# mxy-kit/poisson-ellipse-openmp-mpi-cuda-new

Measured on AMD Instinct MI355X. Metric: grid-point updates/sec (MLUPS) + iters-to-tol, 16384^2 grid at 1/2/4/8 MI355X, higher is better.
Workload: dtype fp64; 1 GPU; model=fictitious-domain Poisson ellipse, Jacobi-PCG, 16384x16384, global_batch=1, seq_len=268402689, parallelism=single, split=auto, comm=self, rccl_graph=False, split_sweep=False, kernel=wave, graph_batch=32, overlap=on, exact=False

## Files before the change

### poisson-ellipse-openmp-mpi-cuda-new_amd/csrc/hip/ca_kernels.hip

```cpp
#include <algorithm>
#include <cmath>
#include <type_traits>
#include <utility>
#include <vector>

#include "pcg1_march.hpp"
#include "pcg_device.hpp"
#include "pmx/common.hpp"
#include "pmx/kernels.hpp"
#include "pmx/spec.hpp"

namespace pmx {

using namespace dev;

namespace {

template <int S>
struct CaShape {
  static constexpr int NB = 2 * S + 1;
  static constexpr int NQ = 6 * S;
  static constexpr int NN = S;
  static constexpr int HE = (S + 1) & ~1;
  static constexpr int WO = 128 - 2 * HE;
  static constexpr int AGES = S + 1 > 3 ? S + 1 : 3;
};

template <int S>
__host__ __device__ constexpr int ca_prod_i(int q) {
  if (q <= 2 * S) return q <= S ? q : (q + 1) / 2;
  q -= 2 * S + 1;
  if (q <= 2 * S - 2) return S + 1 + (q <= S - 1 ? q : (q + 1) / 2);
  q -= 2 * S - 1;
  return q <= S ? q : S;
}
template <int S>
__host__ __device__ constexpr int ca_prod_j(int q) {
  if (q <= 2 * S) return q <= S ? 0 : q / 2;
  q -= 2 * S + 1;
  if (q <= 2 * S - 2) return S + 1 + (q <= S - 1 ? 0 : q / 2);
  q -= 2 * S - 1;
  return q <= S ? S + 1 : S + 1 + (q - S);
}

struct CaK {
  double cxh, cyh, d_in, d_out;
};

__device__ __forceinline__ CaK ca_consts(const DevGeom& G) {
  CaK k;
  const double den = 2.0 * (G.cx + G.cy);
  k.cxh = G.cx / den;
  k.cyh = G.cy / den;
  k.d_in = diag<false>(1.0, 1.0, 1.0, 1.0, G);
  k.d_out = diag<false>(G.inv_eps, G.inv_eps, G.inv_eps, G.inv_eps, G);
  return k;
}

template <typename T>
__device__ __forceinline__ const T* ca_col(const T* row, int c) {
  return reinterpret_cast<const T*>(reinterpret_cast<const char*>(row - 8) + unsigned(c + 8) * unsigned(sizeof(T)));
}
template <typename T>
__device__ __forceinline__ T* ca_col(T* row, int c) {
  return reinterpret_cast<T*>(reinterpret_cast<char*>(row - 8) + unsigned(c + 8) * unsigned(sizeof(T)));
}

template <typename T>
__device__ __forceinline__ void ca_load2(const T* row, int c, int cmax, T (&out)[2]) {
  vload_raw<T, 2>(ca_col(row, min(c, cmax)), out);
}

template <typename T>
__device__ __forceinline__ void ca_store2(T* row, int c, const T (&in)[2], bool all, const bool (&own)[2]) {
  typedef T V __attribute__((ext_vector_type(2)));
  if (all) {
    const V v = {in[0], in[1]};
    __builtin_nontemporal_store(v, reinterpret_cast<V*>(ca_col(row, c)));
  } else {
#pragma unroll
    for (int u = 0; u < 2; ++u)
      if (own[u]) __builtin_nontemporal_store(in[u], ca_col(row, c + u));
  }
}

constexpr int kCaRowOff = 8;

__device__ __forceinline__ int ca_row_cls(const unsigned* tbl, int m) {
  const int r = m + kCaRowOff;
  const unsigned wd = ld_uniform(tbl, r >> 4);
  return int((wd >> (2 * (r & 15))) & 3u);
}

struct CaFaces {
  const double* a;
  const double* b;
  int gh;
};

__device__ __forceinline__ int ca_cmax(const DevGeom& G, const CaFaces& F) {
  return (G.nb & kNbYhi) ? ((G.ny + F.gh - 1) | 1) : G.ny + 1 + (G.ny & 1);
}

__device__ __forceinline__ void ca_faces(const CaFaces& F, const DevGeom& G, int r, int c0, int cmax,
                                         double (&a0)[2], double (&a1)[2], double (&b0)[2], double (&b1)[2]) {
  const int rc = min(max(r, 1 - F.gh), G.nx + F.gh - 1);
  const double* ra = F.a + int64_t(rc) * G.pitch;
  const double* rb = F.b + int64_t(rc) * G.pitch;
  vload<double, 2>(ca_col(ra, min(c0, cmax)), a0);
  vload<double, 2>(ca_col(ra + G.pitch, min(c0, cmax)), a1);
  vload<double, 2>(ca_col(rb, min(c0, cmax)), b0);
  b1[0] = b0[1];
  b1[1] = *ca_col(rb, min(c0 + 2, cmax + 1));
}

__device__ __forceinline__ void ca_lt(int ucls, int r, const double (&c)[2], const double (&im)[2],
                                      const double (&ip)[2], double left, double right, const CaK& K,
                                      const DevGeom& G, const CaFaces& F, int c0, int cmax, double (&out)[2]) {
  const double jm[2] = {left, c[0]}, jp[2] = {c[1], right};
  if (ucls != 0) {
#pragma unroll
    for (int u = 0; u < 2; ++u) out[u] = -__builtin_fma(K.cyh, jm[u] + jp[u], K.cxh * (im[u] + ip[u]));
    return;
  }
  double a0[2], a1[2], b0[2], b1[2];
  ca_faces(F, G, r, c0, cmax, a0, a1, b0, b1);
#pragma unroll
  for (int u = 0; u < 2; ++u) {
    if (a0[u] == a1[u] && a0[u] == b0[u] && a0[u] == b1[u]) {
      out[u] = -__builtin_fma(K.cyh, jm[u] + jp[u], K.cxh * (im[u] + ip[u]));
    } else {
      const double av = apply_a<false>(c[u], im[u], ip[u], jm[u], jp[u], a0[u], a1[u], b0[u], b1[u], G);
      out[u] = av / diag<false>(a0[u], a1[u], b0[u], b1[u], G) - c[u];
    }
  }
}

__device__ __forceinline__ void ca_diag(int ucls, int r, const CaK& K, const DevGeom& G, const CaFaces& F, int c0,
                                        int cmax, double (&d)[2]) {
  if (ucls != 0) {
    d[0] = d[1] = ucls == 1 ? K.d_in : K.d_out;
    return;
  }
  double a0[2], a1[2], b0[2], b1[2];
  ca_faces(F, G, r, c0, cmax, a0, a1, b0, b1);
#pragma unroll
  for (int u = 0; u < 2; ++u) d[u] = diag<false>(a0[u], a1[u], b0[u], b1[u], G);
}

template <int CTRL>
__device__ __forceinline__ double dpp_shift0(double v) {
  const long long b = __double_as_longlong(v);
  const int lo = __builtin_amdgcn_mov_dpp(int(b), CTRL, 0xf, 0xf, true);
  const int hi = __builtin_amdgcn_mov_dpp(int(b >> 32), CTRL, 0xf, 0xf, true);
  return __longlong_as_double((long long)(unsigned)lo | ((long long)hi << 32));
}


__host__ __device__ inline bool ca_tile_fast(const DevGeom& G, int i0, int i1, int j0, int j1, int r, int he, int wo) {
  return j1 == j0 + wo - 1 && G.gi0 + i0 - r >= 1 && G.gi0 + i1 + r <= G.M - 1 && G.gj0 + j0 - he >= 1 &&
         G.gj0 + j0 - he + 127 <= G.N - 1;
}

template <int S, int sl>
__device__ __forceinline__ void ca_gather(const double (&XP)[S + 1][4][2], const double (&XZ)[S][4][2],
                                          double (&Y)[CaShape<S>::NB][2]) {
#pragma unroll
  for (int l = 0; l <= S; ++l) {
    Y[l][0] = XP[l][sl][0];
    Y[l][1] = XP[l][sl][1];
  }
#pragma unroll
  for (int l = 0; l < S; ++l) {
    Y[S + 1 + l][0] = XZ[l][sl][0];
    Y[S + 1 + l][1] = XZ[l][sl][1];
  }
}

template <int NB>
__device__ __forceinline__ double ca_dot(const double (&c)[NB], const double (&Y)[NB][2], int u, double v0) {
#pragma unroll
  for (int i = 0; i < NB; ++i) v0 = __builtin_fma(c[i], Y[i][u], v0);
  return v0;
}

template <int S, int N>
__device__ __forceinline__ void ca_norms(const double (&pa)[S][CaShape<S>::NB], const double (&Y)[CaShape<S>::NB][2],
                                         int u, double (&acc)[N]) {
  acc[0] = __builtin_fma(Y[0][u], Y[0][u], acc[0]);
#pragma unroll
  for (int j = 1; j < S; ++j) {
    double v = 0.0;
#pragma unroll
    for (int i = 0; i <= j; ++i) v = __builtin_fma(pa[j][i], Y[i][u], v);
#pragma unroll
    for (int i = 0; i < j; ++i) v = __builtin_fma(pa[j][S + 1 + i], Y[S + 1 + i][u], v);
    acc[j] = __builtin_fma(v, v, acc[j]);
  }
}

template <typename T, int S, bool UPD>
struct CaRow {
  T p[2], z[2], w[2];
};

template <typename T, int S, bool UPD, bool FAST, int PF, bool REW, int DPF = 0, int HE = CaShape<S>::HE>
__device__ __forceinline__ void ca_march(const DevGeom& G, const DevTables& Tb, const CaK& K,
                                         const T* __restrict__ pin, const T* __restrict__ zin, T* __restrict__ pout,
                                         T* __restrict__ zout, T* __restrict__ w, int i0, int i1, int j0, int j1,
                                         const unsigned* __restrict__ ctbl, const CaFaces& F,
                                         double (&acc)[CaShape<S>::NQ], const double (&ca)[CaShape<S>::NB],
                                         const double (&cb)[CaShape<S>::NB], const double (&cc)[CaShape<S>::NB],
                                         const double (&pa)[S][CaShape<S>::NB], double* dring = nullptr) {
  using Sh = CaShape<S>;
  constexpr int NB = Sh::NB;
  const int64_t P = G.pitch;
  const int lane = threadIdx.x & 63;
  const int c0 = j0 - HE + 2 * lane;
  const int cmax = ca_cmax(G, F);
  bool colin[2], own[2];
#pragma unroll
  for (int u = 0; u < 2; ++u) {
    const int c = c0 + u, g = G.gj0 + c;
    colin[u] = g >= 1 && g <= G.N - 1;
    own[u] = c >= j0 && c <= j1;
  }
  const bool own_all = own[0] && own[1];
  const bool own_any = own[0] || own[1];
  auto interior_row = [&](int m) { return G.gi0 + m >= 1 && G.gi0 + m <= G.M - 1; };

  auto fetch = [&](int m, CaRow<T, S, UPD>& b) {
    const int mc = min(max(m, 1 - F.gh), G.nx + F.gh);
    ca_load2<T>(pin + int64_t(mc) * P, c0, cmax, b.p);
    ca_load2<T>(zin + int64_t(mc) * P, c0, cmax, b.z);
    if constexpr (UPD) {
      const int wc = min(max(m - S, 1 - F.gh), G.nx + F.gh);
      ca_load2<T>(w + int64_t(wc) * P, c0, cmax, b.w);
    }
  };

  static_assert(Sh::AGES <= 4, "ca_march: window deeper than 4 rows");
  double XP[S + 1][4][2], XZ[S][4][2];
#pragma unroll
  for (int l = 0; l <= S; ++l)
#pragma unroll
    for (int a = 0; a < 4; ++a) XP[l][a][0] = XP[l][a][1] = 0.0;
#pragma unroll
  for (int l = 0; l < S; ++l)
#pragma unroll
    for (int a = 0; a < 4; ++a) XZ[l][a][0] = XZ[l][a][1] = 0.0;
  int ch[4] = {0, 0, 0, 0};

  const int mfirst = i0 - S, mlast = i1 + S;
  auto level = [&](auto& X, auto lc, auto qc, int m) {
    constexpr int l = decltype(lc)::value, q = decltype(qc)::value;
    constexpr int sc = (q - l) & 3, sm = (q - l - 1) & 3, sp = (q - l + 1) & 3;
    const int r = m - l;
    const double(&ctr)[2] = X[l - 1][sc];
    const double left = dpp_shift0<kWaveShr1>(ctr[1]);
    const double right = dpp_shift0<kWaveShl1>(ctr[0]);
    double lt[2];
    ca_lt(ch[sc], r, ctr, X[l - 1][sm], X[l - 1][sp], left, right, K, G, F, c0, cmax, lt);
    const bool rin = FAST || interior_row(r);
#pragma unroll
    for (int u = 0; u < 2; ++u) {
      double v;
      if constexpr (l == 1) v = lt[u];
      else v = __builtin_fma(2.0, lt[u], -X[l - 2][sc][u]);
      X[l][sc][u] = (FAST || (rin && colin[u])) ? v : 0.0;
    }
  };

  auto core = [&](auto qc, int m, const CaRow<T, S, UPD>& cur) {
    constexpr int q = decltype(qc)::value;
    ch[q] = ca_row_cls(ctbl, m);
    const bool rin = FAST || interior_row(m);
#pragma unroll
    for (int u = 0; u < 2; ++u) {
      const bool in = FAST || (rin && colin[u]);
      XP[0][q][u] = in ? double(cur.p[u]) : 0.0;
      XZ[0][q][u] = in ? double(cur.z[u]) : 0.0;
    }
    static_for_while<S>([&](auto l1) {
      level(XP, std::integral_constant<int, decltype(l1)::value + 1>{}, qc, m);
      return true;
    });
    static_for_while<S - 1>([&](auto l1) {
      level(XZ, std::integral_constant<int, decltype(l1)::value + 1>{}, qc, m);
      return true;
    });
    const int g = m - S;
    if (g < i0 || g > i1) return;
    constexpr int sg = (q - S) & 3;
    double Y[NB][2];
    ca_gather<S, sg>(XP, XZ, Y);
    if constexpr (!UPD) {
      double d[2];
      ca_diag(ch[sg], g, K, G, F, c0, cmax, d);
#pragma unroll
      for (int u = 0; u < 2; ++u) {
        if (!(FAST || own[u])) continue;
#pragma unroll
        for (int q = 0; q < Sh::NQ; ++q)
          acc[q] = __builtin_fma(Y[ca_prod_i<S>(q)][u], d[u] * Y[ca_prod_j<S>(q)][u], acc[q]);
      }
    } else {
      T pn[2], zn[2], wn[2];
#pragma unroll
      for (int u = 0; u < 2; ++u) {
        const double sp = REW ? 0.0 : ca_dot(ca, Y, u, 0.0), sz = REW ? 0.0 : ca_dot(cb, Y, u, 0.0);
        const double sw = ca_dot(cc, Y, u, double(cur.w[u]));
        pn[u] = static_cast<T>(sp);
        zn[u] = static_cast<T>(sz);
        wn[u] = static_cast<T>(sw);
        if constexpr (!REW) {
          if (FAST || own[u]) ca_norms<S>(pa, Y, u, acc);
        }
      }
      if (FAST ? own_all : own_any) {
        const int64_t o = int64_t(g) * P;
        if constexpr (!REW) {
          ca_store2<T>(pout + o, c0, pn, FAST || own_all, own);
          ca_store2<T>(zout + o, c0, zn, FAST || own_all, own);
        }
        ca_store2<T>(w + o, c0, wn, FAST || own_all, own);
      }
    }
  };

  static_assert(PF == 1 || PF == 3, "ca_march: prefetch depth 1 or 3");
  if constexpr (DPF > 0) {
    static_assert(DPF == 4 && !UPD && FAST && sizeof(T) == 8, "ca_march: LDS-DMA for pass 1 FAST tiles, 4 rows");
    const unsigned voff = unsigned(c0 + 4) * 8u;
    const unsigned lds0 = unsigned(reinterpret_cast<uintptr_t>(dring));
    auto dma_row = [&](int m, int slot) {
      const unsigned l = lds0 + unsigned(slot) * 2048u;
      asm volatile("s_waitcnt lgkmcnt(0)" ::: "memory");
      dma16(pin + int64_t(m) * P - 4, voff, l);
      dma16(zin + int64_t(m) * P - 4, voff, l + 1024u);
    };
    typedef double d2 __attribute__((ext_vector_type(2)));
#pragma unroll
    for (int q = 0; q < DPF; ++q) dma_row(min(mfirst + q, mlast), q);
    bool more = true;
    for (int m = mfirst; more && m <= mlast; m += 4) {
      more = static_for_while<4>([&](auto qc) {
        constexpr int q = decltype(qc)::value;
        if (m + q > mlast) return false;
        wait_vmcnt<(DPF - 1) * 2>();
        const double* sl = dring + q * 256;
        CaRow<T, S, UPD> cur;
        const d2 pv = *reinterpret_cast<const d2*>(sl + 2 * lane);
        const d2 zv = *reinterpret_cast<const d2*>(sl + 128 + 2 * lane);
        cur.p[0] = pv.x;
        cur.p[1] = pv.y;
        cur.z[0] = zv.x;
        cur.z[1] = zv.y;
        dma_row(min(m + q + DPF, mlast), q);
        core(qc, m + q, cur);
        return true;
      });
    }
    wait_vmcnt<0>();
    if constexpr (FAST) {
#pragma unroll
      for (int q = 0; q < Sh::NQ; ++q) acc[q] = own_all ? acc[q] : 0.0;
    }
    return;
  }
  constexpr int NBUF = PF + 1;
  CaRow<T, S, UPD> buf[NBUF];
#pragma unroll
  for (int q = 0; q < PF; ++q) fetch(min(mfirst + q, mlast), buf[q]);
  bool more = true;
  for (int m = mfirst; more && m <= mlast; m += 4) {
    more = static_for_while<4>([&](auto qc) {
      constexpr int q = decltype(qc)::value;
      if (m + q > mlast) return false;
      fetch(min(m + q + PF, mlast), buf[(q + PF) % NBUF]);
      core(qc, m + q, buf[q % NBUF]);
      return true;
    });
  }
  if constexpr (FAST) {
#pragma unroll
    for (int q = 0; q < Sh::NQ; ++q) acc[q] = own_all ? acc[q] : 0.0;
  }
}

constexpr int kCaPfGram = 3, kCaPfUpd = 1, kCaPfFuse = 1;

struct CaPart {
  int part;
  int tiles_i, ti_lo, ti_hi, tj_lo, tj_hi;
};

__device__ __forceinline__ void ca_part_tile(int k, const CaPart& P, int tiles_j, int& ti, int& tj) {
  if (P.part == 0) {
    ti = k / tiles_j;
    tj = k - ti * tiles_j;
    return;
  }
  const int h = P.ti_hi - P.ti_lo, wj = P.tj_hi - P.tj_lo;
  if (P.part == 1) {
    ti = P.ti_lo + k / wj;
    tj = P.tj_lo + k % wj;
    return;
  }
  const int ntop = P.ti_lo * tiles_j;
  if (k < ntop) { ti = k / tiles_j; tj = k % tiles_j; return; }
  k -= ntop;
  const int nbot = (P.tiles_i - P.ti_hi) * tiles_j;
  if (k < nbot) { ti = P.ti_hi + k / tiles_j; tj = k % tiles_j; return; }
  k -= nbot;
  if (k < h * P.tj_lo) { ti = P.ti_lo + k / P.tj_lo; tj = k % P.tj_lo; return; }
  k -= h * P.tj_lo;
  const int wr = tiles_j - P.tj_hi;
  ti = P.ti_lo + k / wr;
  tj = P.tj_hi + k % wr;
}

template <typename T, int S, bool UPD, int MW, bool DMA, int PART>
__global__ void __launch_bounds__(64, MW)
k_ca_sweep(DevGeom G, DevTables Tb, T* w, T* z0, T* z1, T* p0, T* p1, double* __restrict__ partials,
           const PcgState* St, const CaState* C, int TI, int tiles_j, const unsigned* __restrict__ ctbl,
           int cwords, int64_t pbase, CaFaces faces, CaPart part, int ntiles) {
  using Sh = CaShape<S>;
  constexpr int NB = Sh::NB;
  typedef const __attribute__((address_space(4))) PcgState CPS;
  typedef const __attribute__((address_space(4))) CaState CCS;
  const int done = ((CPS*)St)->done;
  const long long blk = ((CCS*)C)->blk;
  const int nupd = ((CCS*)C)->nupd;
  double ca[NB], cb[NB], cc[NB], pa[S][NB];
#pragma unroll
  for (int i = 0; i < NB; ++i) {
    ca[i] = UPD ? ((CCS*)C)->coef[0][i] : 0.0;
    cb[i] = UPD ? ((CCS*)C)->coef[1][i] : 0.0;
    cc[i] = UPD ? ((CCS*)C)->coef[2][i] : 0.0;
#pragma unroll
    for (int j = 0; j < S; ++j) pa[j][i] = UPD ? ((CCS*)C)->pa[j][i] : 0.0;
  }
  if (UPD ? nupd == 0 : done != 0) return;
  int ti = 0, tj = 0;
  ca_part_tile(xcd_remap(blockIdx.x, gridDim.x), part, tiles_j, ti, tj);
  const int id = ti * tiles_j + tj;
  const int i0 = 1 + ti * TI, i1 = min(i0 + TI - 1, G.nx);
  const int j0 = 1 + tj * Sh::WO, j1 = min(j0 + Sh::WO - 1, G.ny);
  const int in = int((UPD ? blk - 1 : blk) & 1);
  const T* pin = in ? p1 : p0;
  const T* zin = in ? z1 : z0;
  T* pout = in ? p0 : p1;
  T* zout = in ? z0 : z1;
  const CaK K = ca_consts(G);
  const int lane = threadIdx.x & 63;
  __shared__ double s_ring[(!UPD && DMA) ? 4 * 256 : 2];
  const unsigned* tbl = ctbl + int64_t(tj) * cwords;
  const bool fast = PART == 1 || ca_tile_fast(G, i0, i1, j0, j1, S, Sh::HE, Sh::WO);
  double acc[Sh::NQ];
#pragma unroll
  for (int q = 0; q < Sh::NQ; ++q) acc[q] = 0.0;
  constexpr int PF = UPD ? kCaPfUpd : kCaPfGram;
#define PMX_CA_MARCH(F, R) \
  ca_march<T, S, UPD, F, PF, R>(G, Tb, K, pin, zin, pout, zout, w, i0, i1, j0, j1, tbl, faces, acc, ca, cb, cc, pa)
  if constexpr (UPD) {
    if (nupd < 0) {
      if constexpr (PART == 1) PMX_CA_MARCH(true, true);
      else if (fast) PMX_CA_MARCH(true, true);
      else PMX_CA_MARCH(false, true);
      return;
    }
  }
  if constexpr (PART == 1) {
    if constexpr (!UPD && DMA && sizeof(T) == 8)
      ca_march<T, S, UPD, true, PF, false, 4>(G, Tb, K, pin, zin, pout, zout, w, i0, i1, j0, j1, tbl, faces, acc, ca,
                                              cb, cc, pa, s_ring);
    else
      PMX_CA_MARCH(true, false);
    goto marched;
  }
  if constexpr (!UPD && DMA && sizeof(T) == 8) {
    if (fast) {
      ca_march<T, S, UPD, true, PF, false, 4>(G, Tb, K, pin, zin, pout, zout, w, i0, i1, j0, j1, tbl, faces, acc, ca,
                                              cb, cc, pa, s_ring);
      goto marched;
    }
  }
  if (fast) PMX_CA_MARCH(true, false);
  else PMX_CA_MARCH(false, false);
marched:
#undef PMX_CA_MARCH
  constexpr int NOUT = UPD ? Sh::NN : Sh::NQ;
#pragma unroll
  for (int q = 0; q + 1 < NOUT; q += 2) wave_sum2_mfma(acc[q], acc[q + 1]);
  if constexpr (NOUT & 1) acc[NOUT - 1] = wave_sum_mfma(acc[NOUT - 1]);
  if (lane == 0) {
#pragma unroll
    for (int q = 0; q < NOUT; ++q) partials[pbase + int64_t(q) * ntiles + id] = acc[q];
  }
}

template <int S>
struct CaFuseShape {
  static constexpr int HE = 2 * S;
  static constexpr int WO = 128 - 2 * HE;
};

template <typename T>
struct CaFRow {
  T p[2], z[2], w[2];
};

template <typename T, int S, bool FAST, int PF, int ROLE>
__device__ __forceinline__ void ca_march_fused(const DevGeom& G, const CaK& K, const T* __restrict__ pin,
                                               const T* __restrict__ zin, T* __restrict__ pout, T* __restrict__ zout,
                                               T* __restrict__ w, int i0, int i1, int j0, int j1,
                                               const unsigned* __restrict__ ctbl, const CaFaces& F,
                                               double (&acc)[CaShape<S>::NQ], double (&nacc)[S],
                                               const double (&ca)[CaShape<S>::NB], const double (&cb)[CaShape<S>::NB],
                                               const double (&cc)[CaShape<S>::NB],
                                               const double (&pa)[S][CaShape<S>::NB], double* ring) {
  using Sh = CaShape<S>;
  constexpr int NB = Sh::NB, HE = CaFuseShape<S>::HE;
  const int64_t P = G.pitch;
  const int lane = threadIdx.x & 63;
  const int c0 = j0 - HE + 2 * lane;
  const int cmax = ca_cmax(G, F);
  bool colin[2], own[2];
#pragma unroll
  for (int u = 0; u < 2; ++u) {
    const int c = c0 + u, g = G.gj0 + c;
    colin[u] = g >= 1 && g <= G.N - 1;
    own[u] = c >= j0 && c <= j1;
  }
  const bool own_all = own[0] && own[1];
  const bool own_any = own[0] || own[1];
  auto interior_row = [&](int m) { return G.gi0 + m >= 1 && G.gi0 + m <= G.M - 1; };
  typedef double d2 __attribute__((ext_vector_type(2)));
  auto sync = [] {
    __builtin_amdgcn_fence(__ATOMIC_RELEASE, "workgroup");
    __builtin_amdgcn_s_barrier();
    __builtin_amdgcn_fence(__ATOMIC_ACQUIRE, "workgroup");
  };

  double XP[S + 1][4][2], XZ[S][4][2];
#pragma unroll
  for (int a = 0; a < 4; ++a)
#pragma unroll
    for (int u = 0; u < 2; ++u) {
#pragma unroll
      for (int l = 0; l <= S; ++l) XP[l][a][u] = 0.0;
#pragma unroll
      for (int l = 0; l < S; ++l) XZ[l][a][u] = 0.0;
    }
  int ch[4] = {0, 0, 0, 0};

  const int mfirst = i0 - 2 * S, mlast = i1 + 2 * S;
  auto level = [&](auto lc, auto qc, int rb, auto& X) {
    constexpr int l = decltype(lc)::value, q = decltype(qc)::value;
    constexpr int sc = (q - l) & 3, sm = (q - l - 1) & 3, sp = (q - l + 1) & 3;
    const int r = rb - l;
    const double(&ctr)[2] = X[l - 1][sc];
    const double left = dpp_shift0<kWaveShr1>(ctr[1]);
    const double right = dpp_shift0<kWaveShl1>(ctr[0]);
    double lt[2];
    ca_lt(ch[sc], r, ctr, X[l - 1][sm], X[l - 1][sp], left, right, K, G, F, c0, cmax, lt);
    const bool rin = FAST || interior_row(r);
#pragma unroll
    for (int u = 0; u < 2; ++u) {
      double v;
      if constexpr (l == 1) v = lt[u];
      else v = __builtin_fma(2.0, lt[u], -X[l - 2][sc][u]);
      X[l][sc][u] = (FAST || (rin && colin[u])) ? v : 0.0;
    }
  };
  auto chains = [&](auto qc, int rb) {
    static_for_while<S>([&](auto l1) {
      level(std::integral_constant<int, decltype(l1)::value + 1>{}, qc, rb, XP);
      return true;
    });
    static_for_while<S - 1>([&](auto l1) {
      level(std::integral_constant<int, decltype(l1)::value + 1>{}, qc, rb, XZ);
      return true;
    });
  };

  if constexpr (ROLE == 0) {
    auto fetch = [&](int m, CaFRow<T>& b) {
      const int mc = min(max(m, 1 - F.gh), G.nx + F.gh);
      ca_load2<T>(pin + int64_t(mc) * P, c0, cmax, b.p);
      ca_load2<T>(zin + int64_t(mc) * P, c0, cmax, b.z);
      const int wc = min(max(m - S, 1 - F.gh), G.nx + F.gh);
      ca_load2<T>(w + int64_t(wc) * P, c0, cmax, b.w);
    };
    auto core = [&](auto qc, int m, const CaFRow<T>& cur) {
      constexpr int q = decltype(qc)::value;
      ch[q] = ca_row_cls(ctbl, m);
      const bool rin = FAST || interior_row(m);
#pragma unroll
      for (int u = 0; u < 2; ++u) {
        const bool in = FAST || (rin && colin[u]);
        XP[0][q][u] = in ? double(cur.p[u]) : 0.0;
        XZ[0][q][u] = in ? double(cur.z[u]) : 0.0;
      }
      chains(qc, m);
      const int g1 = m - S;
      if (g1 < i0 - S) return;
      double Y[NB][2];
      ca_gather<S, (q - S) & 3>(XP, XZ, Y);
      T pn[2], zn[2];
#pragma unroll
      for (int u = 0; u < 2; ++u) {
        pn[u] = static_cast<T>(ca_dot(ca, Y, u, 0.0));
        zn[u] = static_cast<T>(ca_dot(cb, Y, u, 0.0));
      }
      double* sl = ring + (q & 1) * 256;
      *reinterpret_cast<d2*>(sl + 2 * lane) = d2{double(pn[0]), double(pn[1])};
      *reinterpret_cast<d2*>(sl + 128 + 2 * lane) = d2{double(zn[0]), double(zn[1])};
      if (g1 < i0 || g1 > i1) return;
      T wn[2];
#pragma unroll
      for (int u = 0; u < 2; ++u) {
        wn[u] = static_cast<T>(ca_dot(cc, Y, u, double(cur.w[u])));
        if (FAST || own[u]) ca_norms<S>(pa, Y, u, nacc);
      }
      if (FAST ? own_all : own_any) {
        const int64_t o = int64_t(g1) * P;
        ca_store2<T>(pout + o, c0, pn, FAST || own_all, own);
        ca_store2<T>(zout + o, c0, zn, FAST || own_all, own);
        ca_store2<T>(w + o, c0, wn, FAST || own_all, own);
      }
    };
    static_assert(PF == 1 || PF == 3, "ca_march_fused: prefetch depth 1 or 3");
    constexpr int NBUF = PF + 1;
    CaFRow<T> buf[NBUF];
#pragma unroll
    for (int q = 0; q < PF; ++q) fetch(min(mfirst + q, mlast), buf[q]);
    bool more = true;
    for (int m = mfirst; more && m <= mlast; m += 4) {
      more = static_for_while<4>([&](auto qc) {
        constexpr int q = decltype(qc)::value;
        if (m + q > mlast) return false;
        fetch(min(m + q + PF, mlast), buf[(q + PF) % NBUF]);
        core(qc, m + q, buf[q % NBUF]);
        sync();
        return true;
      });
    }
    if constexpr (FAST) {
#pragma unroll
      for (int j = 0; j < S; ++j) nacc[j] = own_all ? nacc[j] : 0.0;
    }
  } else {
    auto core = [&](auto qc, int m) {
      constexpr int q = decltype(qc)::value;
      const int g1 = m - S;
      if (g1 < i0 - S) return;
      constexpr int s1 = (q - S) & 3;
      const double* sl = ring + (q & 1) * 256;
      const d2 pv = *reinterpret_cast<const d2*>(sl + 2 * lane);
      const d2 zv = *reinterpret_cast<const d2*>(sl + 128 + 2 * lane);
      ch[s1] = ca_row_cls(ctbl, g1);
      XP[0][s1][0] = pv.x;
      XP[0][s1][1] = pv.y;
      XZ[0][s1][0] = zv.x;
      XZ[0][s1][1] = zv.y;
      chains(std::integral_constant<int, s1>{}, g1);
      const int g2 = g1 - S;
      if (g2 < i0) return;
      constexpr int s2 = (q - 2 * S) & 3;
      double Y2[NB][2];
      ca_gather<S, s2>(XP, XZ, Y2);
      double d[2];
      ca_diag(ch[s2], g2, K, G, F, c0, cmax, d);
#pragma unroll
      for (int u = 0; u < 2; ++u) {
        if (!(FAST || own[u])) continue;
#pragma unroll
        for (int qq = 0; qq < Sh::NQ; ++qq)
          acc[qq] = __builtin_fma(Y2[ca_prod_i<S>(qq)][u], d[u] * Y2[ca_prod_j<S>(qq)][u], acc[qq]);
      }
    };
    bool more = true;
    for (int m = mfirst; more && m <= mlast; m += 4) {
      more = static_for_while<4>([&](auto qc) {
        constexpr int q = decltype(qc)::value;
        if (m + q > mlast) return false;
        sync();
        core(qc, m + q);
        return true;
      });
    }
    if constexpr (FAST) {
#pragma unroll
      for (int q = 0; q < Sh::NQ; ++q) acc[q] = own_all ? acc[q] : 0.0;
    }
  }
}

template <typename T, int S, int MW, int PART>
__global__ void __launch_bounds__(128, MW)
k_ca_fused(DevGeom G, T* w, T* z0, T* z1, T* p0, T* p1, double* __restrict__ partials, const CaState* C, int TI,
           int tiles_j, const unsigned* __restrict__ ctbl, int cwords, CaFaces faces, CaPart part, int ntiles) {
  using Sh = CaShape<S>;
  using Fs = CaFuseShape<S>;
  constexpr int NB = Sh::NB;
  typedef const __attribute__((address_space(4))) CaState CCS;
  const long long blk = ((CCS*)C)->blk;
  const int nupd = ((CCS*)C)->nupd;
  if (nupd == 0) return;
  const int role = __builtin_amdgcn_readfirstlane(int(threadIdx.x) >> 6);
  double ca[NB], cb[NB], cc[NB], pa[S][NB];
#pragma unroll
  for (int i = 0; i < NB; ++i) {
    ca[i] = ((CCS*)C)->coef[0][i];
    cb[i] = ((CCS*)C)->coef[1][i];
    cc[i] = ((CCS*)C)->coef[2][i];
#pragma unroll
    for (int j = 0; j < S; ++j) pa[j][i] = ((CCS*)C)->pa[j][i];
  }
  int ti = 0, tj = 0;
  ca_part_tile(xcd_remap(blockIdx.x, gridDim.x), part, tiles_j, ti, tj);
  const int id = ti * tiles_j + tj;
  const int i0 = 1 + ti * TI, i1 = min(i0 + TI - 1, G.nx);
  const int j0 = 1 + tj * Fs::WO, j1 = min(j0 + Fs::WO - 1, G.ny);
  const int in = int((blk - 1) & 1);
  T* pin = in ? p1 : p0;
  T* zin = in ? z1 : z0;
  T* pout = in ? p0 : p1;
  T* zout = in ? z0 : z1;
  const CaK K = ca_consts(G);
  const int lane = threadIdx.x & 63;
  const unsigned* tbl = ctbl + int64_t(tj) * cwords;
  const bool fast = PART == 1 || (j1 == j0 + Fs::WO - 1 && G.gi0 + i0 - 2 * S >= 1 && G.gi0 + i1 + 2 * S <= G.M - 1 &&
                                   G.gj0 + j0 - Fs::HE >= 1 && G.gj0 + j0 - Fs::HE + 127 <= G.N - 1);
  double acc[Sh::NQ], nacc[S];
#pragma unroll
  for (int q = 0; q < Sh::NQ; ++q) acc[q] = 0.0;
#pragma unroll
  for (int j = 0; j < S; ++j) nacc[j] = 0.0;
  if (nupd < 0) {
    if (role != 0) return;
    double pz[S][NB] = {};
    if (PART == 1 || fast)
      ca_march<T, S, true, true, kCaPfUpd, true, 0, Fs::HE>(G, DevTables{}, K, pin, zin, pout, zout, w, i0, i1, j0, j1,
                                                            tbl, faces, acc, ca, cb, cc, pz);
    else if constexpr (PART != 1)
      ca_march<T, S, true, false, kCaPfUpd, true, 0, Fs::HE>(G, DevTables{}, K, pin, zin, pout, zout, w, i0, i1, j0,
                                                             j1, tbl, faces, acc, ca, cb, cc, pz);
    return;
  }
  __shared__ double ring[2 * 256];
#define PMX_CAF_MARCH(FA, R)                                                                                       \
  ca_march_fused<T, S, FA, kCaPfFuse, R>(G, K, pin, zin, pout, zout, w, i0, i1, j0, j1, tbl, faces, acc, nacc, ca, \
                                         cb, cc, pa, ring)
  if (role == 0) {
    if (PART == 1 || fast) PMX_CAF_MARCH(true, 0);
    else if constexpr (PART != 1) PMX_CAF_MARCH(false, 0);
#pragma unroll
    for (int j = 0; j + 1 < S; j += 2) wave_sum2_mfma(nacc[j], nacc[j + 1]);
    if constexpr (S & 1) nacc[S - 1] = wave_sum_mfma(nacc[S - 1]);
    if (lane == 0) {
#pragma unroll
      for (int j = 0; j < S; ++j) partials[int64_t(Sh::NQ + j) * ntiles + id] = nacc[j];
    }
  } else {
    if (PART == 1 || fast) PMX_CAF_MARCH(true, 1);
    else if constexpr (PART != 1) PMX_CAF_MARCH(false, 1);
#pragma unroll
    for (int q = 0; q + 1 < Sh::NQ; q += 2) wave_sum2_mfma(acc[q], acc[q + 1]);
    if constexpr (Sh::NQ & 1) acc[Sh::NQ - 1] = wave_sum_mfma(acc[Sh::NQ - 1]);
    if (lane == 0) {
#pragma unroll
      for (int q = 0; q < Sh::NQ; ++q) partials[int64_t(q) * ntiles + id] = acc[q];
    }
  }
#undef PMX_CAF_MARCH
}

__global__ void k_ca_row_classes(DevGeom G, DevTables Tb, int he, int wo, int tiles_j, int cwords, unsigned* out) {
  const int t = int(blockIdx.x * blockDim.x + threadIdx.x);
  if (t >= tiles_j * cwords) return;
  const int tj = t / cwords, wd = t - tj * cwords;
  const int j0 = 1 + tj * wo;
  const int gjlo = max(G.gj0 + j0 - he, 0), gjhi = min(G.gj0 + j0 - he + 127, G.N);
  unsigned bits = 0;
  for (int q = 0; q < 16; ++q) {
    const int m = wd * 16 + q - kCaRowOff;
    const int gi = min(max(G.gi0 + m, 0), G.M);
    RowConst rc;
    for (int k = 0; k < 4; ++k) {
      rc.ca0[k] = Tb.acls[4 * gi + k];
      rc.ca1[k] = Tb.acls[4 * (gi + 1) + k];
      rc.cb[k] = Tb.bcls[4 * gi + k];
    }
    bits |= unsigned(row_class(rc, gjlo, gjhi)) << (2 * q);
  }
  out[t] = bits;
}

__global__ void __launch_bounds__(256) k_ca_faces(DevGeom G, DevTables Tb, double* fa, double* fb, int gh) {
  const int jlo = (G.nb & kNbYlo) ? -8 : -1, jhi = (G.nb & kNbYhi) ? G.ny + gh + 2 : G.ny + 2;
  const int lj = jlo + int(blockIdx.x * blockDim.x + threadIdx.x);
  const int li = 1 - gh + int(blockIdx.y);
  if (lj > jhi) return;
  const int gi = min(max(G.gi0 + li, 0), G.M), gj = min(max(G.gj0 + lj, 0), G.N);
  const int64_t o = int64_t(li) * G.pitch + lj;
  fa[o] = coef_a(Tb, G, gi, gj);
  fb[o] = coef_b(Tb, G, gi, gj);
}

template <typename T>
__global__ void __launch_bounds__(256) k_ca_init(DevGeom G, DevTables Tb, T* z, T* p) {
  const int lj = 1 + int(blockIdx.x * blockDim.x + threadIdx.x);
  const int li = 1 + int(blockIdx.y);
  if (lj > G.ny) return;
  const int gi = G.gi0 + li, gj = G.gj0 + lj;
  const double a0 = coef_a(Tb, G, gi, gj), a1 = coef_a(Tb, G, gi + 1, gj);
  const double b0 = coef_b(Tb, G, gi, gj), b1 = coef_b(Tb, G, gi, gj + 1);
  const int64_t o = int64_t(li) * G.pitch + lj;
  const double v = dirichlet(G, gi, gj) ? 0.0 : double(z[o]) / diag<false>(a0, a1, b0, b1, G);
  z[o] = static_cast<T>(v);
  p[o] = static_cast<T>(v);
}

template <int S, bool RES>
__device__ void ca_finish(const double* t, const double* u, double h, double wdiff, int nmax, bool check_only,
                          PcgState* St, CaState* C) {
  using Sh = CaShape<S>;
  constexpr int NB = Sh::NB;
  C->nupd = 0;
  if (St->done) return;
  if (C->pend_n > 0) {
    const int n = C->pend_n;
    double diff = 0.0;
    for (int j = 0; j < n; ++j) {
      diff = fabs(C->alpha[j]) * sqrt(u[j] * wdiff);
      const bool bad = !(diff == diff);
      if (bad || (!RES && diff < St->delta)) {
        const long long kk = C->pend_k + j + 1;
        if (j + 1 < n) {
          for (int i = 0; i < NB; ++i) C->coef[2][i] = C->pc[j][i] - C->pc[n - 1][i];
          C->nupd = -1;
        }
        St->it = kk;
        St->iters = kk;
        St->diff = diff;
        St->status = bad ? int(Status::kBreakdown) : int(Status::kConverged);
        if (bad) St->nan_flag = 1;
        St->done = 1;
        C->pend_n = 0;
        return;
      }
    }
    St->diff = diff;
    C->pend_n = 0;
    if (C->after_status != 0) {
      St->iters = C->after_iters;
      St->status = C->after_status;
      St->done = 1;
      C->after_status = 0;
      return;
    }
  }
  if (check_only) return;
  const long long k = St->it;
  const long long left = St->max_iter - k;
  if (left <= 0) {
    St->iters = k;
    St->status = int(Status::kMaxIter);
    St->done = 1;
    return;
  }
  const int nm = int(left < nmax ? left : nmax);
  double mu[2 * S + 1], nu[2 * S - 1], rho[2 * S];
  bool nan = false;
  for (int q = 0; q < Sh::NQ; ++q) nan |= !(t[q] == t[q]) || isinf(t[q]);
  for (int m = 0; m <= S; ++m) mu[m] = t[m] * h;
  for (int m = S + 1; m <= 2 * S; ++m) mu[m] = 2.0 * t[m] * h - mu[m & 1];
  for (int m = 0; m < S; ++m) nu[m] = t[2 * S + 1 + m] * h;
  for (int m = S; m <= 2 * S - 2; ++m) nu[m] = 2.0 * t[2 * S + 1 + m] * h - nu[m & 1];
  for (int m = 0; m <= S; ++m) rho[m] = t[4 * S + m] * h;
  for (int b = 1; b < S; ++b) rho[S + b] = 2.0 * t[5 * S + b] * h - rho[S - b];
  double Gm[NB][NB];
  for (int a = 0; a <= S; ++a) {
    for (int b = 0; b <= S; ++b) Gm[a][b] = 0.5 * (mu[a + b] + mu[a > b ? a - b : b - a]);
    for (int b = 0; b < S; ++b)
      Gm[a][S + 1 + b] = Gm[S + 1 + b][a] = 0.5 * (rho[a + b] + rho[a > b ? a - b : b - a]);
  }
  for (int a = 0; a < S; ++a)
    for (int b = 0; b < S; ++b) Gm[S + 1 + a][S + 1 + b] = 0.5 * (nu[a + b] + nu[a > b ? a - b : b - a]);
  auto quad = [&](const double* x, const double* y) {
    double r = 0.0;
    for (int i = 0; i < NB; ++i) {
      double v = 0.0;
      for (int j = 0; j < NB; ++j) v = __builtin_fma(Gm[i][j], y[j], v);
      r = __builtin_fma(x[i], v, r);
    }
    return r;
  };
  auto shiftT = [&](const double* x, double* y) {
    for (int base = 0; base <= S + 1; base += S + 1) {
      const int n = base == 0 ? S + 1 : S;
      for (int r = 0; r < n; ++r) {
        double v = x[base + r];
        if (r >= 1) v += (r == 1 ? 1.0 : 0.5) * x[base + r - 1];
        if (r + 1 < n) v += 0.5 * x[base + r + 1];
        y[base + r] = v;
      }
    }
  };
  double a[NB], b[NB], c[NB], Ta[NB];
  for (int i = 0; i < NB; ++i) a[i] = b[i] = c[i] = 0.0;
  a[0] = 1.0;
  b[S + 1] = 1.0;
  double g = Gm[S + 1][S + 1];
  const bool weighted = St->norm == int(Norm::kWeighted);
  int n = 0;
  for (int j = 0; j < nm; ++j) {
    shiftT(a, Ta);
    const double den = quad(a, Ta);
    if (nan || !(den == den) || !(g == g) || (weighted ? fabs(den) < St->bd_tol : den < St->bd_tol)) {
      C->after_status = int(Status::kBreakdown);
      C->after_iters = k + j + 1;
      if (nan || !(den == den) || !(g == g)) St->nan_flag = 1;
      break;
    }
    const double alpha = g / den;
    for (int i = 0; i < NB; ++i) {
      C->pa[j][i] = a[i];
      c[i] = __builtin_fma(alpha, a[i], c[i]);
      C->pc[j][i] = c[i];
    }
    C->alpha[j] = alpha;
    n = j + 1;
    for (int i = 0; i < NB; ++i) b[i] = __builtin_fma(-alpha, Ta[i], b[i]);
    const double gn = quad(b, b);
    const double beta = gn / g;
    for (int i = 0; i < NB; ++i) a[i] = __builtin_fma(beta, a[i], b[i]);
    g = gn;
    if constexpr (RES) {
      if (g <= St->stop_thr2) {
        C->after_status = int(Status::kConverged);
        C->after_iters = k + j + 1;
        break;
      }
    }
  }
  if constexpr (RES) St->stop_rho = g;
  if (n == 0) {
    St->iters = C->after_iters;
    St->status = C->after_status;
    St->done = 1;
    C->after_status = 0;
    return;
  }
  if (C->after_status == 0 && k + n >= St->max_iter) {
    C->after_status = int(Status::kMaxIter);
    C->after_iters = St->max_iter;
  }
  for (int i = 0; i < NB; ++i) {
    C->coef[0][i] = a[i];
    C->coef[1][i] = b[i];
    C->coef[2][i] = c[i];
  }
  C->nupd = n;
  C->blk += 1;
  C->pend_n = n;
  C->pend_k = k;
  St->it = k + n;
}

template <typename X>
__device__ __forceinline__ void wave_copy(X* dst, const X* src, int lane) {
  static_assert(sizeof(X) % 8 == 0, "wave_copy: whole 8-byte words");
  const unsigned long long* a = reinterpret_cast<const unsigned long long*>(src);
  unsigned long long* b = reinterpret_cast<unsigned long long*>(dst);
  for (int i = lane; i < int(sizeof(X) / 8); i += kWave) b[i] = a[i];
}
__device__ __forceinline__ void wave_lds_sync() {
  __builtin_amdgcn_fence(__ATOMIC_RELEASE, "workgroup");
  __builtin_amdgcn_wave_barrier();
  __builtin_amdgcn_fence(__ATOMIC_ACQUIRE, "workgroup");
}

template <int S, bool RES = false>
__global__ void __launch_bounds__(256)
k_ca_reduce(const double* __restrict__ part, int n, int n2, double h, double wdiff, int nmax, int check_only,
            int finish, PcgState* St, CaState* C, double* chunk, long long* progress) {
  using Sh = CaShape<S>;
  constexpr int NT = Sh::NQ + Sh::NN;
  __shared__ double lds[NT][256 / kWave];
  __shared__ double tot[NT];
  __shared__ int last;
  if (St->done) {
    if (blockIdx.x == 0 && threadIdx.x == 0) C->nupd = 0;
    return;
  }
  const int q0 = check_only ? Sh::NQ : 0;
  const int nb = int(gridDim.x);
  double s[NT];
#pragma unroll
  for (int q = 0; q < NT; ++q) s[q] = 0.0;
  if (!check_only) {
    const int lo = int(int64_t(n) * blockIdx.x / nb), hi = int(int64_t(n) * (blockIdx.x + 1) / nb);
    for (int i = lo + int(threadIdx.x); i < hi; i += 256) {
#pragma unroll
      for (int q = 0; q < Sh::NQ; ++q) s[q] += part[int64_t(q) * n + i];
    }
  }
  {
    const double* p2 = part + int64_t(Sh::NQ) * n;
    const int lo = int(int64_t(n2) * blockIdx.x / nb), hi = int(int64_t(n2) * (blockIdx.x + 1) / nb);
    for (int i = lo + int(threadIdx.x); i < hi; i += 256) {
#pragma unroll
      for (int q = Sh::NQ; q < NT; ++q) s[q] += p2[int64_t(q - Sh::NQ) * n2 + i];
    }
  }
  const int wid = threadIdx.x / kWave, lane = threadIdx.x % kWave;
#pragma unroll
  for (int q = 0; q < NT; ++q) {
    s[q] = wave_sum_mfma(s[q]);
    if (lane == 0) lds[q][wid] = s[q];
  }
  __syncthreads();
  if (nb > 1) {
    if (threadIdx.x == 0) {
#pragma unroll
      for (int q = 0; q < NT; ++q)
        st_publish(chunk + NT * blockIdx.x + q, (lds[q][0] + lds[q][1]) + (lds[q][2] + lds[q][3]));
      last = ticket_arrive_last(&C->ticket, nb);
    }
    __syncthreads();
    if (!last || threadIdx.x >= kWave) return;
    double t[NT];
#pragma unroll
    for (int q = 0; q < NT; ++q) t[q] = 0.0;
    for (int r = 0; r < (nb + kWave - 1) / kWave; ++r) {
      const int c = lane + kWave * r;
#pragma unroll
      for (int q = 0; q < NT; ++q)
        if (q >= q0) t[q] += c < nb ? ld_published(chunk + NT * c + q) : 0.0;
    }
#pragma unroll
    for (int q = 0; q < NT; ++q) {
      t[q] = wave_sum_mfma(t[q]);
      if (lane == 0) tot[q] = t[q];
    }
  } else {
    if (threadIdx.x >= kWave) return;
    if (lane < NT) tot[lane] = (lds[lane][0] + lds[lane][1]) + (lds[lane][2] + lds[lane][3]);
  }
  __builtin_amdgcn_wave_barrier();
  __builtin_amdgcn_fence(__ATOMIC_RELEASE, "wavefront");
  if (finish) {
// ... 380 lines not shown
```

### poisson-ellipse-openmp-mpi-cuda-new_amd/csrc/hip/ca_solver.hip

```cpp
#include <algorithm>
#include <cstring>
#include <functional>
#include <vector>

#include "pmx/common.hpp"
#include "pmx/gpu_solver.hpp"
#include "pmx/trace.hpp"

namespace pmx {

void GpuSubdomainSolver::ca_pass(hipStream_t s, int kind) {
  hipEvent_t wait = ca_frame_wait_;
  ca_frame_wait_ = nullptr;
  auto launch = [&](hipStream_t side) {
    with_storage([&](auto t) {
      using T = decltype(t);
      const Fields<T> F = fields<T>();
      if (kind == 2)
        launch_ca_fused<T>(ca_geom_, F.w, F.r, F.r2, F.p0, F.p1, partials_.get(), ca_state_.get(), ca_tiles_, s, side,
                           wait);
      else
        launch_ca_sweep<T>(ca_geom_, ca_tables_, F.w, F.r, F.r2, F.p0, F.p1, partials_.get(), state_, ca_state_.get(),
                           ca_tiles_, kind == 1, s, side, wait);
    });
  };
  if (ca_side_) {
    HIP_CHECK(hipEventRecord(ca_ev_fork_.get(), s));
    HIP_CHECK(hipStreamWaitEvent(ca_side_.get(), ca_ev_fork_.get(), 0));
    launch(ca_side_.get());
    HIP_CHECK(hipEventRecord(ca_ev_join_.get(), ca_side_.get()));
    HIP_CHECK(hipStreamWaitEvent(s, ca_ev_join_.get(), 0));
  } else {
    launch(nullptr);
  }
  after_launch(s);
}

void GpuSubdomainSolver::drop_side_stream() {
  if (!ca_side_) return;
  HIP_CHECK(hipSetDevice(opt_.device));
  HIP_CHECK(hipStreamSynchronize(ca_side_.get()));
  ca_side_.reset();
  ca_ev_fork_.reset();
  ca_ev_join_.reset();
}

void GpuSubdomainSolver::enqueue_ca_pass(hipStream_t s, bool upd) {
  PMX_CHECK(ca_, "not an s-step solver");
  ca_pass(s, upd ? 1 : 0);
}

void GpuSubdomainSolver::enqueue_ca_fused(hipStream_t s) {
  PMX_CHECK(ca_fused(), "not an s-step solver with the fused pass");
  ca_pass(s, 2);
}

void GpuSubdomainSolver::enqueue_ca_reduce(hipStream_t s, int n, bool check_only, bool finish, bool fused) {
  PMX_CHECK(ca_, "not an s-step solver");
  PMX_CHECK(!fused || ca_fused(), "fused reduction without the fused pass");
  const double wdiff = spec_.norm == Norm::kWeighted ? g_.h1h2 : 1.0;
  const int n1 = fused ? ca_tiles_.ntilesf() : ca_tiles_.ntiles();
  const int n2 = fused ? ca_tiles_.ntilesf() : ca_tiles_.ntiles2();
  launch_ca_reduce(partials_.get(), n1, n2, ca_tiles_.s, g_.h1h2, wdiff, check_only ? 1 : n, check_only, state_,
                   ca_state_.get(), ca_chunk_.get(), s, progress_dev_, finish,
                   spec_.stop == StopRule::kResidual);
  after_launch(s);
  if (!check_only) {
    ++ca_blk_;
    host_k_ += n;
  }
}

void GpuSubdomainSolver::enqueue_ca_finish(hipStream_t s, int n, bool check_only) {
  PMX_CHECK(ca_, "not an s-step solver");
  const double wdiff = spec_.norm == Norm::kWeighted ? g_.h1h2 : 1.0;
  launch_ca_finish(ca_tiles_.s, g_.h1h2, wdiff, check_only ? 1 : n, check_only, state_, ca_state_.get(), s,
                   progress_dev_, spec_.stop == StopRule::kResidual);
  after_launch(s);
}

GpuSubdomainSolver::CaProbe GpuSubdomainSolver::ca_probe(const std::vector<double>& z, const std::vector<double>& p,
                                                         const std::vector<double>& w, const std::vector<double>& coef,
                                                         const std::vector<double>& pa, bool fused, hipStream_t s) {
  PMX_CHECK(ca_ && plan_.elem == 8, "ca_probe: not an fp64 s-step solver");
  PMX_CHECK(!fused || ca_fused(), "ca_probe: the fused pass runs undecomposed grids");
  const int S = ca_tiles_.s, NB = 2 * S + 1, NQ = 6 * S;
  const size_t rows = size_t(sd_.nx + 2 * plan_.gh), cols = size_t(sd_.ny + 2);
  PMX_CHECK(z.size() == rows * cols && p.size() == rows * cols && w.size() == rows * cols,
            "ca_probe: fields must be (nx + 2 gh) x (ny + 2)");
  PMX_CHECK(coef.size() == size_t(3 * NB) && pa.size() == size_t(S * NB), "ca_probe: coefficient shapes");
  HIP_CHECK(hipSetDevice(opt_.device));
  enqueue_init(s);
  HIP_CHECK(hipStreamSynchronize(s));
  auto put = [&](int f, const std::vector<double>& v) {
    HIP_CHECK(hipMemcpy2D(field_ptr(f, 1 - plan_.gh), plan_.row_bytes(), v.data(), cols * 8, cols * 8, rows,
                          hipMemcpyHostToDevice));
  };
  put(1, z);
  put(2, p);
  put(0, w);
  CaProbe out;
  auto sums = [&](int64_t base, int nq, int n) {
    const std::vector<double> h = read_partials(s);
    std::vector<double> r(size_t(nq), 0.0);
    for (int q = 0; q < nq; ++q)
      for (int i = 0; i < n; ++i) r[size_t(q)] += h[size_t(base + int64_t(q) * n + i)];
    return r;
  };
  CaState c{};
  HIP_CHECK(hipMemcpy(&c, ca_state_.get(), sizeof(CaState), hipMemcpyDeviceToHost));
  c.blk = 1;
  c.nupd = S;
  for (int k = 0; k < 3; ++k)
    for (int i = 0; i < NB; ++i) c.coef[k][i] = coef[size_t(k * NB + i)];
  for (int j = 0; j < S; ++j)
    for (int i = 0; i < NB; ++i) c.pa[j][i] = pa[size_t(j * NB + i)];
  if (!fused) {
    enqueue_ca_pass(s, false);
    HIP_CHECK(hipStreamSynchronize(s));
    out.gram = sums(0, NQ, ca_tiles_.ntiles());
    HIP_CHECK(hipMemcpy(ca_state_.get(), &c, sizeof(CaState), hipMemcpyHostToDevice));
    enqueue_ca_pass(s, true);
    HIP_CHECK(hipStreamSynchronize(s));
    out.norms = sums(int64_t(NQ) * ca_tiles_.ntiles(), S, ca_tiles_.ntiles2());
  } else {
    HIP_CHECK(hipMemcpy(ca_state_.get(), &c, sizeof(CaState), hipMemcpyHostToDevice));
    enqueue_ca_fused(s);
    HIP_CHECK(hipStreamSynchronize(s));
    const std::vector<double> gn = sums(0, NQ + S, ca_tiles_.ntilesf());
    out.gram.assign(gn.begin(), gn.begin() + NQ);
    out.norms.assign(gn.begin() + NQ, gn.end());
  }
  auto get = [&](int f) {
    std::vector<double> h(size_t(sd_.nx) * sd_.ny);
    HIP_CHECK(hipMemcpy2D(h.data(), size_t(sd_.ny) * 8, field_ptr(f, 1, 1), plan_.row_bytes(), size_t(sd_.ny) * 8,
                          size_t(sd_.nx), hipMemcpyDeviceToHost));
    return h;
  };
  out.p = get(3);
  out.z = get(4);
  out.w = get(0);
  return out;
}

HaloMsgs GpuSubdomainSolver::ca_halo_msgs(int set) const {
  PMX_CHECK(ca_, "ca_halo_msgs: not an s-step solver");
  HaloMsgs out;
  const int gh = plan_.gh;
  for (int slot = 0; slot < 2; ++slot) {
    if (layout_.peer[slot] < 0) continue;
    const int64_t srow = slot == 0 ? 1 : sd_.nx - gh + 1, rrow = slot == 0 ? 1 - gh : sd_.nx + 1;
    out.m[out.n++] = row_msg(slot, 0, set ? 4 : 1, gh, srow, rrow);
    out.m[out.n++] = row_msg(slot, 1, set ? 3 : 2, gh, srow, rrow);
  }
  return out;
}

void PcgDriver::ca_exchange(std::vector<hipStream_t>& streams) {
  if (direct_) {
    comm_->halo(local_, streams);
    return;
  }
  comm_->before_pack(local_, streams);
  for (size_t i = 0; i < local_.size(); ++i) {
    HIP_CHECK(hipSetDevice(local_[i]->device()));
    local_[i]->enqueue_halo_pack(streams[i]);
  }
  poison(streams);
  comm_->halo(local_, streams);
  for (size_t i = 0; i < local_.size(); ++i) {
    HIP_CHECK(hipSetDevice(local_[i]->device()));
    local_[i]->enqueue_halo_unpack(streams[i]);
  }
  HIP_CHECK(hipSetDevice(local_[0]->device()));
}

int PcgDriver::ca_batch() const {
  const int s = local_[0]->ca_s();
  const int b = graph_batch_ > 0 ? graph_batch_ : 16;
  return (b + s - 1) / s * s;
}

void PcgDriver::enqueue_ca(int64_t n, const std::function<void(int)>& mark) {
  const int s = local_[0]->ca_s();
  HIP_CHECK(hipSetDevice(local_[0]->device()));
  if (n <= 0) return;
  auto mk = [&](int b) {
    if (mark) mark(b);
  };
  auto each = [&](auto&& f) {
    for (size_t i = 0; i < local_.size(); ++i) {
      HIP_CHECK(hipSetDevice(local_[i]->device()));
      f(local_[i], streams_[i]);
    }
    HIP_CHECK(hipSetDevice(local_[0]->device()));
  };
  const bool fused = local_[0]->ca_fused();
  const bool primed = fused && local_[0]->ca_primed();
  auto set_primed = [&](bool v) {
    for (auto* g : local_) g->set_ca_primed(v);
  };
  if (!any_nb_ && local_.size() == 1 && comm_->world_size() == 1) {
    GpuSubdomainSolver* g = local_[0];
    hipStream_t st = streams_[0];
    bool first = true;
    while (n > 0) {
      const int m = int(std::min<int64_t>(s, n));
      if (fused && !first) g->enqueue_ca_fused(st);
      else if (!primed) g->enqueue_ca_pass(st, false);
      if (!(first && primed)) mk(kPhA);
      g->enqueue_ca_reduce(st, m, false, true, fused && !(first && !primed));
      mk(kPhRed);
      if (!fused) {
        g->enqueue_ca_pass(st, true);
        mk(kPhB);
      }
      first = false;
      n -= m;
    }
    if (fused) {
      g->enqueue_ca_fused(st);
      mk(kPhA);
    }
    g->enqueue_ca_reduce(st, 1, true, true, fused);
    mk(kPhRed);
    g->enqueue_ca_pass(st, true);
    mk(kPhB);
    set_primed(fused);
    return;
  }
  const bool ovl = any_nb_ && overlap_ && !comm_streams_.empty() && !mark;
  bool pending = false;
  auto frame_waits = [&](bool on) {
    size_t u = 0;
    for (size_t i = 0; i < local_.size(); ++i) {
      if (i > 0 && streams_[i] != streams_[i - 1]) ++u;
      local_[i]->set_ca_frame_wait(on ? ev_halo_[u] : nullptr);
    }
  };
  const bool ar = comm_->world_size() > 1;
  auto exchange = [&] {
    if (any_nb_ && ovl) {
      for_each_stream([&](size_t i, size_t u) {
        HIP_CHECK(hipEventRecord(ev_packed_[u], streams_[i]));
        HIP_CHECK(hipStreamWaitEvent(comm_streams_[i], ev_packed_[u], 0));
      });
      ca_exchange(comm_streams_);
      for_each_stream([&](size_t i, size_t u) { HIP_CHECK(hipEventRecord(ev_halo_[u], comm_streams_[i])); });
      frame_waits(true);
      pending = true;
    } else if (any_nb_) {
      ca_exchange(streams_);
      mk(kPhHalo);
    }
  };
  bool first = true;
  while (n > 0) {
    const int m = int(std::min<int64_t>(s, n));
    const bool f = fused && !first;
    if (f) each([&](GpuSubdomainSolver* g, hipStream_t st) { g->enqueue_ca_fused(st); });
    else if (!primed) each([&](GpuSubdomainSolver* g, hipStream_t st) { g->enqueue_ca_pass(st, false); });
    if (!(first && primed)) mk(kPhA);
    if (f) exchange();
    each([&](GpuSubdomainSolver* g, hipStream_t st) { g->enqueue_ca_reduce(st, m, false, false, f || primed); });
    mk(kPhRed);
    comm_->allreduce(local_, 3, streams_);
    if (ar) mk(kPhAr);
    each([&](GpuSubdomainSolver* g, hipStream_t st) { g->enqueue_ca_finish(st, m, false); });
    mk(kPhRed);
    if (!fused) {
      each([&](GpuSubdomainSolver* g, hipStream_t st) { g->enqueue_ca_pass(st, true); });
      mk(kPhB);
      exchange();
    }
    first = false;
    n -= m;
  }
  if (fused) {
    each([&](GpuSubdomainSolver* g, hipStream_t st) { g->enqueue_ca_fused(st); });
    mk(kPhA);
    exchange();
  }
  each([&](GpuSubdomainSolver* g, hipStream_t st) { g->enqueue_ca_reduce(st, 1, true, false, fused); });
  mk(kPhRed);
  comm_->allreduce(local_, 3, streams_);
  if (ar) mk(kPhAr);
  each([&](GpuSubdomainSolver* g, hipStream_t st) { g->enqueue_ca_finish(st, 1, true); });
  mk(kPhRed);
  each([&](GpuSubdomainSolver* g, hipStream_t st) { g->enqueue_ca_pass(st, true); });
  mk(kPhB);
  if (pending) {
    for_each_stream([&](size_t i, size_t u) { HIP_CHECK(hipStreamWaitEvent(streams_[i], ev_halo_[u], 0)); });
    frame_waits(false);
  }
  set_primed(fused);
}

int PcgDriver::ca_phase() const {
  return (any_nb_ ? int(local_[0]->ca_blocks() & 1) : 0) + (local_[0]->ca_primed() ? 2 : 0);
}

}
```

Baseline: 295,000 MLUPS.

## Move fused-pass global stores from producer to consumer wave via LDS ring

Result: no change. 296,500 MLUPS, median of 5 (+0.5%).

```diff
diff --git a/poisson-ellipse-openmp-mpi-cuda-new_amd/csrc/hip/ca_kernels.hip b/poisson-ellipse-openmp-mpi-cuda-new_amd/csrc/hip/ca_kernels.hip
--- a/poisson-ellipse-openmp-mpi-cuda-new_amd/csrc/hip/ca_kernels.hip
+++ b/poisson-ellipse-openmp-mpi-cuda-new_amd/csrc/hip/ca_kernels.hip
@@ -57,6 +57,13 @@
   return k;
 }
 
+__device__ __forceinline__ double ca_sgpr(double v) {
+  const long long b = __double_as_longlong(v);
+  const unsigned lo = unsigned(__builtin_amdgcn_readfirstlane(int(b)));
+  const unsigned hi = unsigned(__builtin_amdgcn_readfirstlane(int(b >> 32)));
+  return __longlong_as_double((long long)lo | ((long long)hi << 32));
+}
+
 template <typename T>
 __device__ __forceinline__ const T* ca_col(const T* row, int c) {
   return reinterpret_cast<const T*>(reinterpret_cast<const char*>(row - 8) + unsigned(c + 8) * unsigned(sizeof(T)));
@@ -81,6 +88,25 @@
 #pragma unroll
     for (int u = 0; u < 2; ++u)
       if (own[u]) __builtin_nontemporal_store(in[u], ca_col(row, c + u));
+  }
+}
+
+template <typename T>
+__device__ __forceinline__ void ca_store2_srow(T* first, int lane, const T (&in)[2], bool all, const bool (&own)[2]) {
+  typedef T V __attribute__((ext_vector_type(2)));
+  typedef __attribute__((address_space(1))) char GC;
+  typedef __attribute__((address_space(1))) T GT;
+  typedef __attribute__((address_space(1))) V GV;
+  asm("" : "+s"(first));
+  GC* base = (GC*)reinterpret_cast<char*>(first);
+  const unsigned off = unsigned(lane) * unsigned(2 * sizeof(T));
+  if (all) {
+    const V v = {in[0], in[1]};
+    __builtin_nontemporal_store(v, (GV*)(base + off));
+  } else {
+#pragma unroll
+    for (int u = 0; u < 2; ++u)
+      if (own[u]) __builtin_nontemporal_store(in[u], (GT*)(base + (off + unsigned(u * sizeof(T)))));
   }
 }
 
@@ -511,8 +537,10 @@
   T p[2], z[2], w[2];
 };
 
+constexpr int kCaRingSlot = 3 * 128;
+
 template <typename T, int S, bool FAST, int PF, int ROLE>
-__device__ __forceinline__ void ca_march_fused(const DevGeom& G, const CaK& K, const T* __restrict__ pin,
+__device__ __forceinline__ void ca_march_fused(const DevGeom& G, const CaK& Kv, const T* __restrict__ pin,
                                                const T* __restrict__ zin, T* __restrict__ pout, T* __restrict__ zout,
                                                T* __restrict__ w, int i0, int i1, int j0, int j1,
                                                const unsigned* __restrict__ ctbl, const CaFaces& F,
@@ -522,6 +550,7 @@
                                                const double (&pa)[S][CaShape<S>::NB], double* ring) {
   using Sh = CaShape<S>;
   constexpr int NB = Sh::NB, HE = CaFuseShape<S>::HE;
+  const CaK K = ROLE == 1 ? CaK{ca_sgpr(Kv.cxh), ca_sgpr(Kv.cyh), ca_sgpr(Kv.d_in), ca_sgpr(Kv.d_out)} : Kv;
   const int64_t P = G.pitch;
   const int lane = threadIdx.x & 63;
   const int c0 = j0 - HE + 2 * lane;
@@ -614,7 +643,7 @@
         pn[u] = static_cast<T>(ca_dot(ca, Y, u, 0.0));
         zn[u] = static_cast<T>(ca_dot(cb, Y, u, 0.0));
       }
-      double* sl = ring + (q & 1) * 256;
+      double* sl = ring + (q & 1) * kCaRingSlot;
       *reinterpret_cast<d2*>(sl + 2 * lane) = d2{double(pn[0]), double(pn[1])};
       *reinterpret_cast<d2*>(sl + 128 + 2 * lane) = d2{double(zn[0]), double(zn[1])};
       if (g1 < i0 || g1 > i1) return;
@@ -624,12 +653,7 @@
         wn[u] = static_cast<T>(ca_dot(cc, Y, u, double(cur.w[u])));
         if (FAST || own[u]) ca_norms<S>(pa, Y, u, nacc);
       }
-      if (FAST ? own_all : own_any) {
-        const int64_t o = int64_t(g1) * P;
-        ca_store2<T>(pout + o, c0, pn, FAST || own_all, own);
-        ca_store2<T>(zout + o, c0, zn, FAST || own_all, own);
-        ca_store2<T>(w + o, c0, wn, FAST || own_all, own);
-      }
+      *reinterpret_cast<d2*>(sl + 256 + 2 * lane) = d2{double(wn[0]), double(wn[1])};
     };
     static_assert(PF == 1 || PF == 3, "ca_march_fused: prefetch depth 1 or 3");
     constexpr int NBUF = PF + 1;
@@ -657,7 +681,7 @@
       const int g1 = m - S;
       if (g1 < i0 - S) return;
       constexpr int s1 = (q - S) & 3;
-      const double* sl = ring + (q & 1) * 256;
+      const double* sl = ring + (q & 1) * kCaRingSlot;
       const d2 pv = *reinterpret_cast<const d2*>(sl + 2 * lane);
       const d2 zv = *reinterpret_cast<const d2*>(sl + 128 + 2 * lane);
       ch[s1] = ca_row_cls(ctbl, g1);
@@ -665,6 +689,16 @@
       XP[0][s1][1] = pv.y;
       XZ[0][s1][0] = zv.x;
       XZ[0][s1][1] = zv.y;
+      if (g1 >= i0 && g1 <= i1 && (FAST ? own_all : own_any)) {
+        const d2 wv = *reinterpret_cast<const d2*>(sl + 256 + 2 * lane);
+        const T pn[2] = {static_cast<T>(pv.x), static_cast<T>(pv.y)};
+        const T zn[2] = {static_cast<T>(zv.x), static_cast<T>(zv.y)};
+        const T wn[2] = {static_cast<T>(wv.x), static_cast<T>(wv.y)};
+        const int64_t o = int64_t(g1) * P + (j0 - HE);
+        ca_store2_srow<T>(pout + o, lane, pn, FAST || own_all, own);
+        ca_store2_srow<T>(zout + o, lane, zn, FAST || own_all, own);
+        ca_store2_srow<T>(w + o, lane, wn, FAST || own_all, own);
+      }
       chains(std::integral_constant<int, s1>{}, g1);
       const int g2 = g1 - S;
       if (g2 < i0) return;
@@ -750,7 +784,7 @@
                                                              j1, tbl, faces, acc, ca, cb, cc, pz);
     return;
   }
-  __shared__ double ring[2 * 256];
+  __shared__ double ring[2 * kCaRingSlot];
 #define PMX_CAF_MARCH(FA, R)                                                                                       \
   ca_march_fused<T, S, FA, kCaPfFuse, R>(G, K, pin, zin, pout, zout, w, i0, i1, j0, j1, tbl, faces, acc, nacc, ca, \
                                          cb, cc, pa, ring)
diff --git a/poisson-ellipse-openmp-mpi-cuda-new_amd/csrc/hip/ca_solver.hip b/poisson-ellipse-openmp-mpi-cuda-new_amd/csrc/hip/ca_solver.hip
--- a/poisson-ellipse-openmp-mpi-cuda-new_amd/csrc/hip/ca_solver.hip
+++ b/poisson-ellipse-openmp-mpi-cuda-new_amd/csrc/hip/ca_solver.hip
@@ -82,7 +82,8 @@
 GpuSubdomainSolver::CaProbe GpuSubdomainSolver::ca_probe(const std::vector<double>& z, const std::vector<double>& p,
                                                          const std::vector<double>& w, const std::vector<double>& coef,
                                                          const std::vector<double>& pa, bool fused, hipStream_t s) {
-  PMX_CHECK(ca_ && plan_.elem == 8, "ca_probe: not an fp64 s-step solver");
+  PMX_CHECK(ca_, "ca_probe: not an s-step solver");
+  const size_t e = plan_.elem;
   PMX_CHECK(!fused || ca_fused(), "ca_probe: the fused pass runs undecomposed grids");
   const int S = ca_tiles_.s, NB = 2 * S + 1, NQ = 6 * S;
   const size_t rows = size_t(sd_.nx + 2 * plan_.gh), cols = size_t(sd_.ny + 2);
@@ -93,7 +94,9 @@
   enqueue_init(s);
   HIP_CHECK(hipStreamSynchronize(s));
   auto put = [&](int f, const std::vector<double>& v) {
-    HIP_CHECK(hipMemcpy2D(field_ptr(f, 1 - plan_.gh), plan_.row_bytes(), v.data(), cols * 8, cols * 8, rows,
+    const std::vector<float> v32(e == 4 ? v.begin() : v.end(), v.end());
+    const void* src = e == 4 ? static_cast<const void*>(v32.data()) : v.data();
+    HIP_CHECK(hipMemcpy2D(field_ptr(f, 1 - plan_.gh), plan_.row_bytes(), src, cols * e, cols * e, rows,
                           hipMemcpyHostToDevice));
   };
   put(1, z);
@@ -133,8 +136,11 @@
   }
   auto get = [&](int f) {
     std::vector<double> h(size_t(sd_.nx) * sd_.ny);
-    HIP_CHECK(hipMemcpy2D(h.data(), size_t(sd_.ny) * 8, field_ptr(f, 1, 1), plan_.row_bytes(), size_t(sd_.ny) * 8,
+    std::vector<float> h32(e == 4 ? h.size() : 0);
+    void* dst = e == 4 ? static_cast<void*>(h32.data()) : h.data();
+    HIP_CHECK(hipMemcpy2D(dst, size_t(sd_.ny) * e, field_ptr(f, 1, 1), plan_.row_bytes(), size_t(sd_.ny) * e,
                           size_t(sd_.nx), hipMemcpyDeviceToHost));
+    if (e == 4) h.assign(h32.begin(), h32.end());
     return h;
   };
   out.p = get(3);
```
